# AzureLeon1/DiffSpectra

Measured on AMD Instinct MI355X. Metric: molecules/sec, 1000-step QM9S all-spectra sampling (partial run), higher is better.
Workload: dtype f32 (GEMMs as split-fp16 x3 MFMA with fp32 accumulate; fp32-level accuracy, parity gates unchanged)

## Files before the change

diffspectra_amd/csrc/ds_device.h:

```cpp
#pragma once
#include <hip/hip_runtime.h>
#include <stdint.h>

typedef float f32x16 __attribute__((ext_vector_type(16)));
typedef float f32x2 __attribute__((ext_vector_type(2)));
typedef _Float16 h4 __attribute__((ext_vector_type(4)));
typedef _Float16 h8 __attribute__((ext_vector_type(8)));
typedef float f32x4 __attribute__((ext_vector_type(4)));

#define DS_LDP 4

__device__ __forceinline__ float ds_silu(float x) { return __fdividef(x, 1.0f + __expf(-x)); }
__device__ __forceinline__ float ds_tanh(float x) {
  const float e = __builtin_amdgcn_exp2f(x * 2.8853900817779268f);
  return fmaf(-2.0f, __builtin_amdgcn_rcpf(e + 1.0f), 1.0f);
}
__device__ __forceinline__ f32x2 ds_tanh2_prescaled(f32x2 t) {
  f32x2 e;
  e.x = __builtin_amdgcn_exp2f(t.x); e.y = __builtin_amdgcn_exp2f(t.y);
  const f32x2 d = e + 1.0f;
  f32x2 r;
  r.x = __builtin_amdgcn_rcpf(d.x); r.y = __builtin_amdgcn_rcpf(d.y);
  return r * -2.0f + 1.0f;
}
// ... 191 lines not shown
  int voff;
  int kstride;
  int pstride;
};
__device__ __forceinline__ WStreamH wstream_h(const float* __restrict__ Wh, int N, int K, int col0) {
  const int lane = threadIdx.x & 63;
  WStreamH w;
  const unsigned long long pw = reinterpret_cast<unsigned long long>(Wh);
  const unsigned long long pu = (static_cast<unsigned long long>(__builtin_amdgcn_readfirstlane(static_cast<int>(pw >> 32))) << 32) |
                                static_cast<unsigned int>(__builtin_amdgcn_readfirstlane(static_cast<int>(pw)));
  w.rsrc = __builtin_amdgcn_make_buffer_rsrc(reinterpret_cast<float*>(pu), 0, 0x7fffffff, 0x00020000);
  w.voff = ((lane >> 5) * N + col0 + (lane & 31)) << 4;
  w.kstride = N << 5;
  w.pstride = (K >> 4) * w.kstride;
  return w;
}
__device__ __forceinline__ h8 wload_h(const WStreamH& w, int plane, int kb) {
  return __builtin_bit_cast(h8, __builtin_amdgcn_raw_buffer_load_b128(w.rsrc, w.voff, plane * w.pstride + kb * w.kstride, 0));
}

template <int MT, bool TRANS = false, int UNROLL = 4, bool XPF = true>
__device__ __forceinline__ void wave_mma_h(const _Float16* X, int K_tile, const float* __restrict__ Wh, int N, int K, int col0,
                                           int kb0, int kb1, f32x16 (&hi)[MT], f32x16 (&lo)[MT], int xkb0 = 0) {
  const int lane = threadIdx.x & 63, r = lane & 31, hh = lane >> 5;
  const int ldh = 2 * K_tile + 8;
  const WStreamH ws = wstream_h(Wh, N, K, col0);
  const _Float16* xr = X + r * ldh + 8 * hh - xkb0 * 16;
  h8 w1 = wload_h(ws, 0, kb0), w2 = wload_h(ws, 1, kb0);
  h8 xa[MT][2];
#pragma unroll
  for (int m = 0; m < MT; ++m) {
    xa[m][0] = *reinterpret_cast<const h8*>(xr + m * 32 * ldh + kb0 * 16);
    xa[m][1] = *reinterpret_cast<const h8*>(xr + m * 32 * ldh + K_tile + kb0 * 16);
  }
#pragma unroll UNROLL
  for (int kb = kb0; kb < kb1; ++kb) {
    const int kn = min(kb + 1, kb1 - 1);
    const h8 w1n = wload_h(ws, 0, kn), w2n = wload_h(ws, 1, kn);
    h8 xn[MT][2];
    if (XPF) {
#pragma unroll
      for (int m = 0; m < MT; ++m) {
        xn[m][0] = *reinterpret_cast<const h8*>(xr + m * 32 * ldh + kn * 16);
        xn[m][1] = *reinterpret_cast<const h8*>(xr + m * 32 * ldh + K_tile + kn * 16);
      }
    }
    __builtin_amdgcn_sched_barrier(0);
#pragma unroll
    for (int m = 0; m < MT; ++m) {
      if (TRANS) {
        hi[m] = __builtin_amdgcn_mfma_f32_32x32x16_f16(w1, xa[m][0], hi[m], 0, 0, 0);
        lo[m] = __builtin_amdgcn_mfma_f32_32x32x16_f16(w1, xa[m][1], lo[m], 0, 0, 0);
        lo[m] = __builtin_amdgcn_mfma_f32_32x32x16_f16(w2, xa[m][0], lo[m], 0, 0, 0);
      } else {
        hi[m] = __builtin_amdgcn_mfma_f32_32x32x16_f16(xa[m][0], w1, hi[m], 0, 0, 0);
        lo[m] = __builtin_amdgcn_mfma_f32_32x32x16_f16(xa[m][1], w1, lo[m], 0, 0, 0);
        lo[m] = __builtin_amdgcn_mfma_f32_32x32x16_f16(xa[m][0], w2, lo[m], 0, 0, 0);
      }
    }
    w1 = w1n; w2 = w2n;
#pragma unroll
    for (int m = 0; m < MT; ++m) {
      if (XPF) { xa[m][0] = xn[m][0]; xa[m][1] = xn[m][1]; }
      else {
        xa[m][0] = *reinterpret_cast<const h8*>(xr + m * 32 * ldh + kn * 16);
        xa[m][1] = *reinterpret_cast<const h8*>(xr + m * 32 * ldh + K_tile + kn * 16);
      }
    }
  }
}
constexpr int DS_MMA_XD = 1;
template <int PF>
struct WRingH {
  h8 w1[PF], w2[PF];
};
template <int PF>
__device__ __forceinline__ void wring_h(WRingH<PF>& ring, const WStreamH& ws, int kb0) {
#pragma unroll
  for (int i = 0; i < PF; ++i) {
    ring.w1[i] = wload_h(ws, 0, kb0 + i); ring.w2[i] = wload_h(ws, 1, kb0 + i);
    __builtin_amdgcn_sched_barrier(0);
  }
}
template <int MT, bool TRANS, int NKB, int PF, int XD = DS_MMA_XD>
__device__ __forceinline__ void wave_mma_h_deep(const _Float16* X, int K_tile, const WStreamH& ws, WRingH<PF>& ring, int kb0,
                                                f32x16 (&hi)[MT], f32x16 (&lo)[MT], int xkb0 = 0) {
  static_assert(PF <= NKB && XD <= NKB, "ring deeper than the product");
  const int lane = threadIdx.x & 63, r = lane & 31, hh = lane >> 5;
  const int ldh = 2 * K_tile + 8;
  const _Float16* xr = X + r * ldh + 8 * hh + (kb0 - xkb0) * 16;
  h8 xq[XD][MT][2];
#pragma unroll
  for (int d = 0; d < XD; ++d)
#pragma unroll
    for (int m = 0; m < MT; ++m) {
      xq[d][m][0] = *reinterpret_cast<const h8*>(xr + m * 32 * ldh + d * 16);
      xq[d][m][1] = *reinterpret_cast<const h8*>(xr + m * 32 * ldh + K_tile + d * 16);
    }
#pragma unroll
  for (int i = 0; i < NKB; ++i) {
    __builtin_amdgcn_sched_barrier(0);
    const h8 w1 = ring.w1[i % PF], w2 = ring.w2[i % PF];
    h8 xa[MT][2];
#pragma unroll
    for (int m = 0; m < MT; ++m) { xa[m][0] = xq[i % XD][m][0]; xa[m][1] = xq[i % XD][m][1]; }
#define DS_MMA_(ACC, WV, XV) ACC = TRANS ? __builtin_amdgcn_mfma_f32_32x32x16_f16(WV, XV, ACC, 0, 0, 0) : __builtin_amdgcn_mfma_f32_32x32x16_f16(XV, WV, ACC, 0, 0, 0)
#pragma unroll
    for (int m = 0; m < MT; ++m) DS_MMA_(lo[m], w1, xa[m][1]);
#pragma unroll
    for (int m = 0; m < MT; ++m) DS_MMA_(hi[m], w1, xa[m][0]);
#pragma unroll
    for (int m = 0; m < MT; ++m) DS_MMA_(lo[m], w2, xa[m][0]);
#undef DS_MMA_
    if (i + PF < NKB) {
      ring.w1[i % PF] = wload_h(ws, 0, kb0 + i + PF);
      ring.w2[i % PF] = wload_h(ws, 1, kb0 + i + PF);
    }
    if (i + XD < NKB) {
#pragma unroll
      for (int m = 0; m < MT; ++m) {
        xq[i % XD][m][0] = *reinterpret_cast<const h8*>(xr + m * 32 * ldh + (i + XD) * 16);
        xq[i % XD][m][1] = *reinterpret_cast<const h8*>(xr + m * 32 * ldh + K_tile + (i + XD) * 16);
      }
    }
    __builtin_amdgcn_sched_barrier(0);
  }
}
template <int MT, bool TRANS, int NKB, int PF>
__device__ __forceinline__ void wave_mma_h_deep_t2(const _Float16* X, int K_tile, const WStreamH& wsA, const WStreamH& wsB,
                                                   WRingH<PF>& ringA, WRingH<PF>& ringB, int kb0, f32x16 (&hiA)[MT], f32x16 (&loA)[MT],
                                                   f32x16 (&hiB)[MT], f32x16 (&loB)[MT], int xkb0 = 0) {
  static_assert(PF <= NKB, "ring deeper than the product");
  const int lane = threadIdx.x & 63, r = lane & 31, hh = lane >> 5;
  const int ldh = 2 * K_tile + 8;
  const _Float16* xr = X + r * ldh + 8 * hh + (kb0 - xkb0) * 16;
  h8 xa[MT][2];
#pragma unroll
  for (int m = 0; m < MT; ++m) {
    xa[m][0] = *reinterpret_cast<const h8*>(xr + m * 32 * ldh);
    xa[m][1] = *reinterpret_cast<const h8*>(xr + m * 32 * ldh + K_tile);
  }
#define DS_MMA_(ACC, WV, XV) ACC = TRANS ? __builtin_amdgcn_mfma_f32_32x32x16_f16(WV, XV, ACC, 0, 0, 0) : __builtin_amdgcn_mfma_f32_32x32x16_f16(XV, WV, ACC, 0, 0, 0)
#pragma unroll
  for (int i = 0; i < NKB; ++i) {
    const int in = i + 1 < NKB ? i + 1 : i;
    h8 xn[MT][2];
#pragma unroll
    for (int m = 0; m < MT; ++m) {
      xn[m][0] = *reinterpret_cast<const h8*>(xr + m * 32 * ldh + in * 16);
      xn[m][1] = *reinterpret_cast<const h8*>(xr + m * 32 * ldh + K_tile + in * 16);
    }
    __builtin_amdgcn_sched_barrier(0);
    const h8 a1 = ringA.w1[i % PF], a2 = ringA.w2[i % PF], b1 = ringB.w1[i % PF], b2 = ringB.w2[i % PF];
#pragma unroll
    for (int m = 0; m < MT; ++m) { DS_MMA_(loA[m], a1, xa[m][1]); DS_MMA_(loB[m], b1, xa[m][1]); }
#pragma unroll
    for (int m = 0; m < MT; ++m) { DS_MMA_(hiA[m], a1, xa[m][0]); DS_MMA_(hiB[m], b1, xa[m][0]); }
#pragma unroll
    for (int m = 0; m < MT; ++m) { DS_MMA_(loA[m], a2, xa[m][0]); DS_MMA_(loB[m], b2, xa[m][0]); }
    if (i + PF < NKB) {
      ringA.w1[i % PF] = wload_h(wsA, 0, kb0 + i + PF); ringA.w2[i % PF] = wload_h(wsA, 1, kb0 + i + PF);
      ringB.w1[i % PF] = wload_h(wsB, 0, kb0 + i + PF); ringB.w2[i % PF] = wload_h(wsB, 1, kb0 + i + PF);
    }
    __builtin_amdgcn_sched_barrier(0);
#pragma unroll
    for (int m = 0; m < MT; ++m) { xa[m][0] = xn[m][0]; xa[m][1] = xn[m][1]; }
  }
#undef DS_MMA_
}
template <int MT, bool TRANS, int NKB, int PF>
__device__ __forceinline__ void wave_mma_h_ring_t2(const _Float16* X, int K_tile, const WStreamH& wsA, const WStreamH& wsB, int kb0,
                                                   f32x16 (&hiA)[MT], f32x16 (&loA)[MT], f32x16 (&hiB)[MT], f32x16 (&loB)[MT], int xkb0 = 0) {
  WRingH<PF> ringA, ringB;
#pragma unroll
  for (int i = 0; i < PF; ++i) {
    ringA.w1[i] = wload_h(wsA, 0, kb0 + i); ringA.w2[i] = wload_h(wsA, 1, kb0 + i);
    ringB.w1[i] = wload_h(wsB, 0, kb0 + i); ringB.w2[i] = wload_h(wsB, 1, kb0 + i);
    __builtin_amdgcn_sched_barrier(0);
  }
  wave_mma_h_deep_t2<MT, TRANS, NKB, PF>(X, K_tile, wsA, wsB, ringA, ringB, kb0, hiA, loA, hiB, loB, xkb0);
}

template <int MT, bool TRANS, int NKB, int PF>
__device__ __forceinline__ void wave_mma_h_ring(const _Float16* X, int K_tile, const float* __restrict__ Wh, int N, int K, int col0,
                                                int kb0, f32x16 (&hi)[MT], f32x16 (&lo)[MT], int xkb0 = 0) {
  const WStreamH ws = wstream_h(Wh, N, K, col0);
  WRingH<PF> ring;
  wring_h<PF>(ring, ws, kb0);
  wave_mma_h_deep<MT, TRANS, NKB, PF>(X, K_tile, ws, ring, kb0, hi, lo, xkb0);
}
template <int MT>
__device__ __forceinline__ void split_finish(f32x16 (&hi)[MT], const f32x16 (&lo)[MT]) {
#pragma unroll
  for (int m = 0; m < MT; ++m)
#pragma unroll
    for (int i = 0; i < 16; ++i) hi[m][i] = fmaf(lo[m][i], 1.0f / 2048.0f, hi[m][i]);
}

template <int MT>
__device__ __forceinline__ void acc_zero(f32x16 (&acc)[MT]) {
#pragma unroll
  for (int m = 0; m < MT; ++m)
#pragma unroll
    for (int i = 0; i < 16; ++i) acc[m][i] = 0.0f;
}

// ... 89 lines not shown
```

diffspectra_amd/csrc/ds_kernels.hip:

```cpp
#include <hip/hip_runtime.h>
#include <math.h>
#include <stdint.h>
#include <stdio.h>
#include <stdlib.h>

#include <atomic>
#include <mutex>
#include <utility>
#include <vector>

#include "../../include/diffspectra_hip.h"
#include "ds_device.h"
#include "ds_train_common.h"

#define ADAC DS_ADA_COLS
constexpr int DS_NODE_PF = 8;
constexpr int DS_NODE_PF2 = 4;
constexpr int DS_QKV_PF = 4;
constexpr int DS_TWO_STREAM_MAX_PAIRS = 400000;

#ifdef DS_STAMPS
#define DS_STAMP_INIT()                                                                                 \
  unsigned long long _sa[16] = {0, 0, 0, 0, 0, 0, 0, 0, 0, 0, 0, 0, 0, 0, 0, 0};                        \
  unsigned long long _t0 = __builtin_amdgcn_s_memtime()
// ... 96 lines not shown
      const int d = c.L.node_dense[row];
      if (k < 6) v = xh[(size_t)d * 9 + 3 + k];
      else if (k < 12) v = cond_x ? cond_x[(size_t)d * 9 + 3 + (k - 6)] : 0.0f;
      else if (k < 15) v = xh[(size_t)d * 9 + (k - 12)];
    }
    in[rr][k] = v;
  }
  __syncthreads();
  const float* W = GW(c, DS_GW_NODE_EMB_W);
  float w[12];
#pragma unroll
  for (int k = 0; k < 12; ++k) w[k] = wp_at(W, 256, k, col);
  const float bias = GW(c, DS_GW_NODE_EMB_B)[col];
#pragma unroll
  for (int rr = 0; rr < R; ++rr) {
    const int row = row0 + rr;
    if (row >= c.L.Nn) break;
    float acc = 0.0f;
#pragma unroll
    for (int k = 0; k < 12; ++k) acc += in[rr][k] * w[k];
    acc += bias;
    c.ws.h[(size_t)row * 256 + col] = acc;
    c.ws.atom_hids[(size_t)row * 768 + col] = acc;
    if (col < 4) c.ws.pos[(size_t)row * 4 + col] = col < 3 ? in[rr][12 + col] : 0.0f;
  }
}

__global__ __launch_bounds__(256) void k_pair_init(Ctx c, const float* __restrict__ edge_x, const float* __restrict__ cond_x,
                                                   const float* __restrict__ cond_edge_x) {
  ds_fp16_saturate();
  constexpr int T = 64;
  __shared__ __attribute__((aligned(16))) float X[T][72 + DS_LDP];
  __shared__ __attribute__((aligned(16))) float xs[T];
  const int tid = threadIdx.x, row0 = blockIdx.x * T;
  const bool use_rbf = (cond_x != nullptr) && (c.ws.flags[0] != 0);
  if (tid < T) {
    const int p = row0 + tid;
    float x = 0.0f;
    float e0 = 0, e1 = 0, c0 = 0, c1 = 0;
    if (p < c.L.Pp) {
      const int da = c.L.node_dense[c.L.pair_a[p]], db = c.L.node_dense[c.L.pair_b[p]];
      const int m = c.L.pair_mol[p];
      const size_t eidx = ((size_t)da * c.L.N + (db - m * c.L.N)) * 2;
      e0 = edge_x[eidx]; e1 = edge_x[eidx + 1];
      if (cond_x != nullptr) {
        c0 = cond_edge_x[eidx]; c1 = cond_edge_x[eidx + 1];
        const float* pa = cond_x + (size_t)da * 9;
        const float* pb = cond_x + (size_t)db * 9;
        const float dx = pa[0] - pb[0], dy = pa[1] - pb[1], dz = pa[2] - pb[2];
        const float d2 = dx * dx + dy * dy + dz * dz;
        const float* ad = c.ws.ada + (size_t)m * ADAC + DS_ADA_TOP;
        x = use_rbf ? d2 * (ad[0] + 1.0f) + ad[1] : d2;
      }
    }
    X[tid][0] = e0; X[tid][1] = e1; X[tid][2] = c0; X[tid][3] = c1;
    X[tid][68] = 0.0f; X[tid][69] = 0.0f; X[tid][70] = 0.0f; X[tid][71] = 0.0f;
    xs[tid] = x;
  }
  __syncthreads();
  const float* mean = GW(c, DS_GW_RBF_MEAN);
  const float* stdv = GW(c, DS_GW_RBF_STD);
  const float* astd = GW(c, DS_GW_RBF_ASTD);
  for (int idx = tid; idx < T * 64; idx += 256) {
    const int row = idx >> 6, k = idx & 63;
    float v = 0.0f;
    if (row0 + row < c.L.Pp) v = use_rbf ? rbf_feature(xs[row], k, mean, stdv, astd) : xs[row];
    X[row][4 + k] = v;
  }
  __syncthreads();
  const float* bias = GW(c, DS_GW_EDGE_EMB_B);
  const int Pp = c.L.Pp;
  float* e = c.ws.e;
  float* hid = c.ws.edge_hids;
  tile_gemm<2, 1>(&X[0][0], 72 + DS_LDP, 72, GW(c, DS_GW_EDGE_EMB_W), 64, 2, [&](int row, int col, float v) {
    const int p = row0 + row;
    if (p < Pp) {
      const float y = v + bias[col];
      e[(size_t)p * 64 + col] = y;
      hid[(size_t)p * 192 + col] = y;
    }
  });
}

__global__ __launch_bounds__(256) void k_edge_geom(Ctx c, int blk) {
  ds_fp16_saturate();
  constexpr int T = 64, LDH = 2 * 128 + 8;
  __shared__ __attribute__((aligned(16))) _Float16 Xh[T][LDH];
  __shared__ __attribute__((aligned(16))) float Y[T][64 + DS_LDP];
  __shared__ __attribute__((aligned(16))) float xs[T];
  __shared__ int rmol[T];
  const int tid = threadIdx.x, row0 = blockIdx.x * T;
  const int kf = tid & 63, rbp = tid >> 6;
  const float mk = kf ? BW(c, blk, DS_BW_RBF_MEAN)[kf - 1] : 0.0f;
  const float sk = kf ? BW(c, blk, DS_BW_RBF_STD)[kf - 1] : 1.0f;
  const float ak = kf ? BW(c, blk, DS_BW_RBF_ASTD)[kf - 1] : 1.0f;
  float ev[16];
#pragma unroll
  for (int j = 0; j < 16; ++j) ev[j] = c.ws.e[(size_t)min(row0 + rbp + 4 * j, c.L.Pp - 1) * 64 + kf];
  if (tid < T) {
    const int p = row0 + tid;
    float x = 0.0f;
    int m = 0;
    if (p < c.L.Pp) {
      m = c.L.pair_mol[p];
      const float* pa = c.ws.pos + (size_t)c.L.pair_a[p] * 4;
      const float* pb = c.ws.pos + (size_t)c.L.pair_b[p] * 4;
      const float dx = pa[0] - pb[0], dy = pa[1] - pb[1], dz = pa[2] - pb[2];
      const float d2 = dx * dx + dy * dy + dz * dz;
      const float* ad = c.ws.ada + (size_t)m * ADAC + blk * DS_ADA_BLOCK_STRIDE + DS_ADA_DIST;
      x = d2 * (ad[0] + 1.0f) + ad[1];
    }
    xs[tid] = x;
    rmol[tid] = m;
    if (p < c.L.Pp) c.ws.dist[p] = x;
  }
  __syncthreads();
  float4 lsh[4], lsc[4];
  {
    const float* ade = c.ws.ada + blk * DS_ADA_BLOCK_STRIDE + DS_ADA_EDGE;
    const int lane = tid & 63, wv = tid >> 6;
#pragma unroll
    for (int j = 0; j < 4; ++j) {
      const float* am = ade + (size_t)rmol[16 * wv + 4 * j + (lane >> 4)] * ADAC;
      lsh[j] = reinterpret_cast<const float4*>(am)[lane & 15];
      lsc[j] = reinterpret_cast<const float4*>(am + 64)[lane & 15];
    }
  }
  {
    const int k = kf, rb = rbp;
    const float rsk = __builtin_amdgcn_rcpf(sk), rak = __builtin_amdgcn_rcpf(ak);
    const int Pp = c.L.Pp;
#pragma unroll
    for (int j = 0; j < 16; ++j) {
      const int row = rb + 4 * j, p = row0 + row;
      const float x = xs[row];
      const float z = (x - mk) * rsk;
      float v = k ? __expf(-0.5f * (z * z)) * rak : x;
      if (p >= Pp) { v = 0.0f; ev[j] = 0.0f; }
      split_store1(&Xh[row][0], 128, k, v);
      split_store1(&Xh[row][0], 128, 64 + k, ev[j]);
    }
  }
  {
    const int wv = tid >> 6, mt = wv >> 1, cc = wv & 1, lane = tid & 63;
    const WStreamH wse = wstream_h(BW(c, blk, DS_BW_EDGE_EMB_H), 64, 128, cc * 32);
    WRingH<8> ring;
    wring_h<8>(ring, wse, 0);
    const float bcol = BW(c, blk, DS_BW_EDGE_EMB_B)[cc * 32 + (lane & 31)];
    __syncthreads();
    f32x16 acc[1], lo[1];
#pragma unroll
    for (int i = 0; i < 16; ++i) acc[0][i] = bcol;
    acc_zero<1>(lo);
    wave_mma_h_deep<1, false, 8, 8>(&Xh[mt * 32][0], 128, wse, ring, 0, acc, lo);
    split_finish<1>(acc, lo);
#pragma unroll
    for (int i = 0; i < 16; ++i) Y[mt * 32 + acc_row(i, lane >> 5)][cc * 32 + (lane & 31)] = acc[0][i];
  }
  __syncthreads();
  {
    const int lane = tid & 63, wv = tid >> 6;
    _Float16* ye = reinterpret_cast<_Float16*>(c.ws.ye);
#pragma unroll
    for (int j = 0; j < 4; ++j) {
      const int row = 16 * wv + 4 * j + (lane >> 4);
      const float4 v = ln_mod_reg64(reinterpret_cast<const float4*>(&Y[row][0])[lane & 15], lsh[j], lsc[j]);
      if (row0 + row < c.L.Pp) split_store4(ye + (size_t)(row0 + row) * 128, 64, 4 * (lane & 15), v);
    }
  }
}

template <int NW>
__global__ __launch_bounds__(NW * 64) void k_node_qkv(Ctx c, int blk) {
  ds_fp16_saturate();
  constexpr int NT = NW * 64;
  constexpr int T = 64;
  constexpr int LDH = 2 * 256 + 8;
  __shared__ __attribute__((aligned(16))) _Float16 Xh[T][LDH];
  __shared__ int rmol[T];
  const int tid = threadIdx.x, row0 = blockIdx.x * T, col0 = blockIdx.y * 384;
  if (tid < T) rmol[tid] = (row0 + tid < c.L.Nn) ? c.L.node_mol[row0 + tid] : 0;
  __syncthreads();
  {
    const float* adn = c.ws.ada + blk * DS_ADA_BLOCK_STRIDE + DS_ADA_NODE;
    const int lane = tid & 63, wv = tid >> 6, g = lane >> 4, j = lane & 15;
    static_assert(NT == 256, "four waves x 16 rows");
#pragma unroll
    for (int half = 0; half < 2; ++half) {
      float4 v[2][4], sh[2][4], sc[2][4];
#pragma unroll
      for (int ps = 0; ps < 2; ++ps) {
        const int row = 16 * wv + 8 * half + 4 * ps + g;
        const float4* hp = reinterpret_cast<const float4*>(c.ws.h + (size_t)min(row0 + row, c.L.Nn - 1) * 256) + j;
        const float4* ap = reinterpret_cast<const float4*>(adn + (size_t)rmol[row] * ADAC) + j;
#pragma unroll
        for (int u = 0; u < 4; ++u) {
          v[ps][u] = hp[16 * u];
          sh[ps][u] = ap[16 * u];
          sc[ps][u] = ap[64 + 16 * u];
        }
      }
#pragma unroll
      for (int ps = 0; ps < 2; ++ps) {
        const int row = 16 * wv + 8 * half + 4 * ps + g;
        ln_mod_quad256(v[ps], sh[ps], sc[ps]);
#pragma unroll
        for (int u = 0; u < 4; ++u)
          split_store4(&Xh[row][0], 256, 64 * u + 4 * j, row0 + row < c.L.Nn ? v[ps][u] : make_float4(0, 0, 0, 0));
      }
    }
  }
  __syncthreads();
  const float* bias = BW(c, blk, DS_BW_QKV_B) + col0;
  float* qkv = c.ws.qkv + (size_t)row0 * 768 + col0;
  const int valid = c.L.Nn - row0, wave = tid >> 6;
  for (int ch = wave; ch < 12; ch += NW) {
    asm volatile("" ::: "memory");
    const float b = bias[ch * 32 + (tid & 31)];
    f32x16 acc[2], lo[2];
#pragma unroll
    for (int m = 0; m < 2; ++m)
#pragma unroll
      for (int i = 0; i < 16; ++i) acc[m][i] = b;
    acc_zero<2>(lo);
    wave_mma_h_ring<2, false, 16, DS_QKV_PF>(&Xh[0][0], 256, BW(c, blk, DS_BW_QKV_H), 768, 256, col0 + ch * 32, 0, acc, lo);
    split_finish<2>(acc, lo);
    acc_store<2, 768>(acc, qkv + ch * 32, valid, [](int, float v) { return v; });
  }
}

__global__ __launch_bounds__(1024) void k_attn_fused(Ctx c, int blk) {
  ds_fp16_saturate();
  DS_STAMP_INIT();
  constexpr int NT = 1024, QS = 512 + 32, LDT = 256 + 4, LDY = 2 * 64 + 8, CR = 32, MAXP = DS_MAX_ATOMS * (DS_MAX_ATOMS - 1) / 2;
  __shared__ __attribute__((aligned(16))) float QK[DS_MAX_ATOMS * QS];
  __shared__ __attribute__((aligned(16))) float Tt[2][CR][LDT];
  __shared__ __attribute__((aligned(16))) _Float16 Yc[2][CR][LDY];
  __shared__ __attribute__((aligned(16))) float AL[2][CR][32];
  __shared__ int PT[(MAXP + 15) & ~15];
  __shared__ int VT[32][32];
  static_assert(DS_MAX_ATOMS <= 32 && MAXP <= 511 - CR, "visit table packing");
  static_assert(DS_MAX_ATOMS * 128 <= 4 * NT && DS_MAX_ATOMS * 64 <= 2 * NT && MAXP <= NT, "single-pass staging");
  const int tid = threadIdx.x, wave = tid >> 6, lane = tid & 63, hh = lane >> 5;
  int n0, n, p0, P;
  if (c.L.mol_by_size) {
    const int4 r = reinterpret_cast<const int4*>(c.L.mol_by_size)[blockIdx.x];
    n0 = r.x; n = r.y; p0 = r.z; P = r.w;
  } else {
    const int m = blockIdx.x;
    n0 = c.L.node_off[m]; n = c.L.node_off[m + 1] - n0;
    p0 = c.L.pair_off[m]; P = c.L.pair_off[m + 1] - p0;
// ... 1033 lines not shown
    for (int u = 0; u < 8; ++u) {
      const int idx = i0 + u * 256, row = idx / 192, k4 = idx - row * 192;
      v[u] = reinterpret_cast<const float4*>(c.ws.atom_hids + (size_t)min(row0 + row, Nn - 1) * 768)[k4];
    }
#pragma unroll
    for (int u = 0; u < 8; ++u) {
      const int idx = i0 + u * 256, row = idx / 192, k4 = idx - row * 192;
      split_store4(&X[row][0], 768, 4 * k4, row0 + row < Nn ? v[u] : make_float4(0, 0, 0, 0));
    }
  }
  __syncthreads();
  {
    const float* b = GW(c, DS_GW_NP0_B);
    for (int ch = wave; ch < 8; ch += 4) {
      asm volatile("" ::: "memory");
      const int col = ch * 32 + (tid & 31), hhf = (tid & 63) >> 5;
      const float bc = b[col];
      f32x16 acc[1], lo[1];
#pragma unroll
      for (int i = 0; i < 16; ++i) acc[0][i] = bc;
      acc_zero<1>(lo);
      wave_mma_h_ring<1, false, 48, 8>(&X[0][0], 768, GW(c, DS_GW_NP0_H), 256, 768, ch * 32, 0, acc, lo);
      split_finish<1>(acc, lo);
#pragma unroll
      for (int i = 0; i < 16; ++i) split_store1(&Y1[acc_row(i, hhf)][0], 256, col, ds_silu(acc[0][i]));
    }
  }
  __syncthreads();
  {
    const float* b = GW(c, DS_GW_NP2_B);
    const int col = wave * 32 + (tid & 31), hhf = (tid & 63) >> 5;
    const float bc = b[col];
    f32x16 acc[1], lo[1];
#pragma unroll
    for (int i = 0; i < 16; ++i) acc[0][i] = bc;
    acc_zero<1>(lo);
    wave_mma_h_ring<1, false, 16, 8>(&Y1[0][0], 256, GW(c, DS_GW_NP2_H), 128, 256, wave * 32, 0, acc, lo);
    split_finish<1>(acc, lo);
#pragma unroll
    for (int i = 0; i < 16; ++i) Y2[acc_row(i, hhf)][col] = ds_silu(acc[0][i]);
  }
  __syncthreads();
  {
    const float* b = GW(c, DS_GW_NP4_B);
    const float bc = b[min((int)(threadIdx.x & 31), 5)];
    tile_gemm<1, 1>(&Y2[0][0], 128 + DS_LDP, 128, GW(c, DS_GW_NP4_W), 32, 1, [&](int row, int col, float v) {
      if (col < 6 && dn[row] >= 0) out_xh[(size_t)dn[row] * 9 + 3 + col] = v + bc;
    });
  }
}

__global__ __launch_bounds__(256) void k_edge_readout(Ctx c, float* __restrict__ out_edge) {
  ds_fp16_saturate();
  const int tid = threadIdx.x, wave = tid >> 6, lane = tid & 63, r = lane & 31, hh = lane >> 5;
  const int Pp = c.L.Pp;
  const int row0 = (blockIdx.x * 4 + wave) * 32;
  if (row0 >= Pp) return;
  const int p = min(row0 + r, Pp - 1);
  const bool valid = row0 + r < Pp;
  const int pa = c.L.pair_a[p], pb = c.L.pair_b[p], pm = c.L.pair_mol[p];
  h8 x1[12], x2[12];
  {
    const float4* src = reinterpret_cast<const float4*>(c.ws.edge_hids + (size_t)p * 192 + 8 * hh);
#pragma unroll
    for (int g4 = 0; g4 < 3; ++g4) {
      float4 v[4][2];
#pragma unroll
      for (int u = 0; u < 4; ++u) { v[u][0] = src[(g4 * 4 + u) * 4]; v[u][1] = src[(g4 * 4 + u) * 4 + 1]; }
#pragma unroll
      for (int u = 0; u < 4; ++u) {
        const float xs[8] = {v[u][0].x, v[u][0].y, v[u][0].z, v[u][0].w, v[u][1].x, v[u][1].y, v[u][1].z, v[u][1].w};
#pragma unroll
        for (int t = 0; t < 8; ++t) {
          const _Float16 a1 = (_Float16)xs[t];
          x1[g4 * 4 + u][t] = a1;
          x2[g4 * 4 + u][t] = (_Float16)((xs[t] - (float)a1) * 2048.0f);
        }
      }
    }
  }
  const int da = c.L.node_dense[pa], db = c.L.node_dense[pb];
  const int mN = pm * c.L.N;
  const size_t oab = ((size_t)da * c.L.N + (db - mN)) * 2, oba = ((size_t)db * c.L.N + (da - mN)) * 2;
  for (int ch = 0; ch < 2; ++ch) {
    const int g0 = ch == 0 ? DS_GW_EX0_W : DS_GW_ET0_W;
    const float* b0 = GW(c, g0 + 1);
    const float* b2 = GW(c, g0 + 3);
    const uint4* W2 = reinterpret_cast<const uint4*>(GW(c, ch == 0 ? DS_GW_EX2_C : DS_GW_ET2_C)) + lane;
    f32x16 a2, a2lo;
#pragma unroll
    for (int q = 0; q < 4; ++q) {
      const float4 bb = *reinterpret_cast<const float4*>(b2 + 8 * q + 4 * hh);
      a2[4 * q] = bb.x; a2[4 * q + 1] = bb.y; a2[4 * q + 2] = bb.z; a2[4 * q + 3] = bb.w;
    }
#pragma unroll
    for (int i = 0; i < 16; ++i) a2lo[i] = 0.0f;
#pragma unroll
    for (int hc = 0; hc < 2; ++hc) {
      asm volatile("" ::: "memory");
      const WStreamH ws0 = wstream_h(GW(c, ch == 0 ? DS_GW_EX0_H : DS_GW_ET0_H), 64, 192, hc * 32);
      WRingH<6> ring;
      wring_h<6>(ring, ws0, 0);
      f32x16 a1, a1lo;
#pragma unroll
      for (int q = 0; q < 4; ++q) {
        const float4 bb = *reinterpret_cast<const float4*>(b0 + hc * 32 + 8 * q + 4 * hh);
        a1[4 * q] = bb.x; a1[4 * q + 1] = bb.y; a1[4 * q + 2] = bb.z; a1[4 * q + 3] = bb.w;
      }
#pragma unroll
      for (int i = 0; i < 16; ++i) a1lo[i] = 0.0f;
#pragma unroll
      for (int kb = 0; kb < 12; ++kb) {
        const h8 w1 = ring.w1[kb % 6], w2 = ring.w2[kb % 6];
        a1lo = __builtin_amdgcn_mfma_f32_32x32x16_f16(w1, x2[kb], a1lo, 0, 0, 0);
        a1 = __builtin_amdgcn_mfma_f32_32x32x16_f16(w1, x1[kb], a1, 0, 0, 0);
        a1lo = __builtin_amdgcn_mfma_f32_32x32x16_f16(w2, x1[kb], a1lo, 0, 0, 0);
        if (kb + 6 < 12) { ring.w1[kb % 6] = wload_h(ws0, 0, kb + 6); ring.w2[kb % 6] = wload_h(ws0, 1, kb + 6); }
        __builtin_amdgcn_sched_barrier(0);
      }
#pragma unroll
      for (int i = 0; i < 16; ++i) a1[i] = fmaf(a1lo[i], 1.0f / 2048.0f, a1[i]);
#pragma unroll
      for (int s_ = 0; s_ < 2; ++s_) {
        h8 y1, y2;
#pragma unroll
        for (int j = 0; j < 8; j += 2) {
          f32x2 v;
          v.x = a1[8 * s_ + j]; v.y = a1[8 * s_ + j + 1];
          v = ds_silu2(v);
          y1[j] = (_Float16)v.x; y1[j + 1] = (_Float16)v.y;
          y2[j] = (_Float16)((v.x - (float)y1[j]) * 2048.0f); y2[j + 1] = (_Float16)((v.y - (float)y1[j + 1]) * 2048.0f);
        }
        const h8 w1 = __builtin_bit_cast(h8, W2[((0 * 2 + hc) * 2 + s_) * 64]);
        const h8 w2 = __builtin_bit_cast(h8, W2[((1 * 2 + hc) * 2 + s_) * 64]);
        a2 = __builtin_amdgcn_mfma_f32_32x32x16_f16(w1, y1, a2, 0, 0, 0);
        a2lo = __builtin_amdgcn_mfma_f32_32x32x16_f16(w1, y2, a2lo, 0, 0, 0);
        a2lo = __builtin_amdgcn_mfma_f32_32x32x16_f16(w2, y1, a2lo, 0, 0, 0);
      }
    }
    const float* W4 = GW(c, g0 + 4);
    f32x2 s2 = {0.0f, 0.0f};
#pragma unroll
    for (int i = 0; i < 16; i += 2) {
      f32x2 v;
      v.x = fmaf(a2lo[i], 1.0f / 2048.0f, a2[i]); v.y = fmaf(a2lo[i + 1], 1.0f / 2048.0f, a2[i + 1]);
      v = ds_silu2(v);
      const f32x2 w = {wp_at(W4, 32, acc_row(i, hh), 0), wp_at(W4, 32, acc_row(i + 1, hh), 0)};
      s2 = __builtin_elementwise_fma(w, v, s2);
    }
    const float part = s2.x + s2.y;
    const auto sw = __builtin_amdgcn_permlane32_swap(__float_as_uint(part), __float_as_uint(part), false, false);
    const float val = (__uint_as_float(sw[0]) + __uint_as_float(sw[1])) + GW(c, g0 + 5)[0];
    if (valid && hh == 0) {
      out_edge[oab + ch] = val;
      out_edge[oba + ch] = val;
    }
  }
}

__global__ void k_final_pos(Ctx c, float* __restrict__ out_xh) {
  const int m = blockIdx.x * blockDim.x + threadIdx.x;
  if (m >= c.L.B) return;
  const int n0 = c.L.node_off[m], n = c.L.node_off[m + 1] - n0;
  const bool nan = c.ws.flags[1] != 0;
  float sx = 0.0f, sy = 0.0f, sz = 0.0f;
  for (int a = 0; a < n; ++a) {
    const float* pp = c.ws.pos + (size_t)(n0 + a) * 4;
    if (!nan) { sx += pp[0]; sy += pp[1]; sz += pp[2]; }
  }
  const float fn = (float)n;
  for (int a = 0; a < n; ++a) {
    const float* pp = c.ws.pos + (size_t)(n0 + a) * 4;
    float* o = out_xh + (size_t)c.L.node_dense[n0 + a] * 9;
    const float px = nan ? 0.0f : pp[0], py = nan ? 0.0f : pp[1], pz = nan ? 0.0f : pp[2];
    o[0] = px - sx / fn; o[1] = py - sy / fn; o[2] = pz - sz / fn;
  }
}

__global__ void k_temb_finish(Ctx c, const float* __restrict__ tm3, int tm3_rows, const float* __restrict__ ctx) {
  ds_fp16_saturate();
  const size_t i = (size_t)blockIdx.x * blockDim.x + threadIdx.x;
  if (i >= (size_t)c.L.B * 1024) return;
  const size_t b = i >> 10, col = i & 1023;
  float v = tm3[(tm3_rows == 1 ? 0 : b) * 1024 + col];
  if (ctx) v += ctx[i];
  split_store1(reinterpret_cast<_Float16*>(c.ws.temb_silu) + b * 2048, 1024, (int)col, ds_silu(v));
}

__global__ __launch_bounds__(256) void k_gemm_ada(const _Float16* __restrict__ A, const float* __restrict__ Wh, const float* __restrict__ bias,
                                                  float* __restrict__ C, int ldc, int M, int K, int N) {
  ds_fp16_saturate();
  constexpr int T = 64, KC = 64, LDH = 2 * KC + 8, MT = T / 32;
  __shared__ __attribute__((aligned(16))) _Float16 X[2][T][LDH];
  const int tid = threadIdx.x, wave = tid >> 6;
  const int row0 = blockIdx.x * T;
  const int col0 = (blockIdx.y * 4 + wave) * 32;
  const bool active = col0 < N;
  const int nchunks = K / KC;
  float4 st0, st1, st2, st3;
  const int srow = tid >> 4, spiece = tid & 15;
  const size_t scol = (size_t)(spiece >> 3) * K + (spiece & 7) * 8;
  auto fetch = [&](int kc) {
    const _Float16* base = A + scol + kc * KC;
    st0 = *reinterpret_cast<const float4*>(base + (size_t)min(row0 + srow, M - 1) * 2 * K);
    st1 = *reinterpret_cast<const float4*>(base + (size_t)min(row0 + srow + 16, M - 1) * 2 * K);
    st2 = *reinterpret_cast<const float4*>(base + (size_t)min(row0 + srow + 32, M - 1) * 2 * K);
    st3 = *reinterpret_cast<const float4*>(base + (size_t)min(row0 + srow + 48, M - 1) * 2 * K);
  };
  auto stash = [&](int buf) {
    *reinterpret_cast<float4*>(&X[buf][srow][spiece * 8]) = st0;
    *reinterpret_cast<float4*>(&X[buf][srow + 16][spiece * 8]) = st1;
    *reinterpret_cast<float4*>(&X[buf][srow + 32][spiece * 8]) = st2;
    *reinterpret_cast<float4*>(&X[buf][srow + 48][spiece * 8]) = st3;
  };
  f32x16 acc[MT], lo[MT];
  acc_zero<MT>(acc);
  acc_zero<MT>(lo);
  const WStreamH wsw = wstream_h(Wh, N, K, active ? col0 : 0);
  WRingH<4> ring;
  wring_h<4>(ring, wsw, 0);
  fetch(0);
  stash(0);
  __syncthreads();
  for (int kc = 0; kc < nchunks; ++kc) {
    const int cur = kc & 1;
    if (kc + 1 < nchunks) fetch(kc + 1);
    if (active) wave_mma_h_deep<MT, false, 4, 4>(&X[cur][0][0], KC, wsw, ring, kc * 4, acc, lo, kc * 4);
    if (kc + 1 < nchunks) { wring_h<4>(ring, wsw, kc * 4 + 4); stash(cur ^ 1); }
    __syncthreads();
  }
  if (!active) return;
  split_finish<MT>(acc, lo);
  const int lane = tid & 63, r = lane & 31, hh = lane >> 5, col = col0 + r;
  const float bcol = bias ? bias[col] : 0.0f;
  const unsigned long long pw = reinterpret_cast<unsigned long long>(C + (size_t)row0 * ldc + col0);
  const unsigned long long pu = (static_cast<unsigned long long>(__builtin_amdgcn_readfirstlane(static_cast<int>(pw >> 32))) << 32) |
                                static_cast<unsigned int>(__builtin_amdgcn_readfirstlane(static_cast<int>(pw)));
  const __amdgpu_buffer_rsrc_t rc = __builtin_amdgcn_make_buffer_rsrc(reinterpret_cast<float*>(pu), 0, 0x7fffffff, 0x00020000);
// ... 428 lines not shown
    if (kc + 1 < nchunks) fetch(kc + 1);
    const float* wp = g.Wp + (size_t)(kc * (KC / 8)) * 2 * g.Npad * 4;
    if (active) wave_mma<4>(&X[cur][0][0], LD, wp, g.Npad, col0, 0, KC / 8, acc, 0, &bf);
    if (kc + 1 < nchunks) {
      stash(cur ^ 1);
      bf = bfrag_load(wp + (size_t)(KC / 8) * 2 * g.Npad * 4, g.Npad, active ? col0 : 0, 0, 8);
    }
    __syncthreads();
  }
  if (!active) return;
  {
    const int lane = tid & 63, r = lane & 31, hh = lane >> 5, col = col0 + r;
    const bool colok = col < g.N;
    const float bcol = (g.bias && colok) ? g.bias[col] : 0.0f;
    const float csc = (g.cs && colok) ? g.cs[col] : 1.0f, csh = (g.cs && colok) ? g.csh[col] : 0.0f;
    const unsigned long long pw = reinterpret_cast<unsigned long long>(g.C + (size_t)row0 * g.ldc + col0);
    const unsigned long long pu = (static_cast<unsigned long long>(__builtin_amdgcn_readfirstlane(static_cast<int>(pw >> 32))) << 32) |
                                  static_cast<unsigned int>(__builtin_amdgcn_readfirstlane(static_cast<int>(pw)));
    const __amdgpu_buffer_rsrc_t rc = __builtin_amdgcn_make_buffer_rsrc(reinterpret_cast<float*>(pu), 0, 0x7fffffff, 0x00020000);
    const int voff = (4 * hh * g.ldc + r) * 4, rowb = g.ldc * 4;
#pragma unroll
    for (int m = 0; m < 4; ++m)
#pragma unroll
      for (int i = 0; i < 16; ++i) {
        const int row = m * 32 + (i & 3) + 8 * (i >> 2), gr = row0 + row + 4 * hh;
        if (gr < g.M && colok) {
          float v = ds_act<ACT>(acc[m][i] + bcol);
          if (g.R) v += g.R[(size_t)(g.r_grp_rows > 0 ? gr % g.r_grp_rows : gr) * g.ldr + col];
          if (g.cs) v = v * csc + csh;
          __builtin_amdgcn_raw_buffer_store_b32(__float_as_uint(v), rc, voff, row * rowb, 0);
        }
      }
  }
}

int gemm_dispatch(const GemmArgs& g, int act, hipStream_t s) {
  if (!g.A || !g.Wp || !g.C || g.M <= 0 || g.K <= 0 || g.N <= 0 || (g.cs && !g.csh)) return DS_ERR_ARG;
  const bool big = g.M >= 512 && g.a_grp_rows <= 0 && g.c_grp_rows <= 0 && g.K % 64 == 0 && g.lda % 4 == 0 &&
                   (reinterpret_cast<uintptr_t>(g.A) & 15) == 0;
  using Kernel = void (*)(GemmArgs);
  static constexpr Kernel tile128[4] = {k_gemm_big<0>, k_gemm_big<1>, k_gemm_big<2>, k_gemm_big<3>};
  static constexpr Kernel tile64[4] = {k_gemm<0>, k_gemm<1>, k_gemm<2>, k_gemm<3>};
  if (act < 0 || act > 3) return DS_ERR_ARG;
  const int rows = big ? 128 : 64;
  hipLaunchKernelGGL(big ? tile128[act] : tile64[act], dim3((g.M + rows - 1) / rows, (g.Npad + 127) / 128), dim3(256), 0, s, g);
  return DST_CHECK_LAUNCH();
}

int gemm_simple(const float* A, int64_t lda, const float* Wp, const float* bias, float* C, int64_t ldc, int M, int K, int N,
                int act, int a_silu, hipStream_t s) {
  GemmArgs g{};
  g.A = A; g.lda = lda; g.Wp = Wp; g.bias = bias; g.C = C; g.ldc = ldc; g.M = M; g.K = K; g.N = N;
  g.Npad = (N + 31) & ~31; g.a_silu = a_silu;
  return gemm_dispatch(g, act, s);
}

enum ProfSlot { PROF_EDGE_GEOM = 0, PROF_NODE_QKV = 1, PROF_ATTN = 2, PROF_NODE_UPDATE = 3, PROF_EDGE_UPDATE = 4, PROF_EQUI_PAIRS = 5 };
struct ProfState {
  int kernel = -1;
  int every = 1;
  long long seen = 0;
  std::vector<std::pair<hipEvent_t, hipEvent_t>> pool;
  size_t used = 0;
};
ProfState g_prof;

struct ProfScope {
  hipStream_t s;
  bool on = false;
  ProfScope(int kernel, hipStream_t st) : s(st) {
    if (g_prof.kernel != kernel) return;
    if ((g_prof.seen++ % g_prof.every) != 0 || g_prof.used >= g_prof.pool.size()) return;
    on = true;
    (void)hipEventRecord(g_prof.pool[g_prof.used].first, s);
  }
  ~ProfScope() {
    if (on) (void)hipEventRecord(g_prof.pool[g_prof.used++].second, s);
  }
};

void launch_edge_geom(const Ctx& c, int blk, hipStream_t s) {
  if (c.L.Pp <= 0) return;
  ProfScope ps(PROF_EDGE_GEOM, s);
  hipLaunchKernelGGL(k_edge_geom, dim3((c.L.Pp + 63) / 64), dim3(256), 0, s, c, blk);
}
void launch_node_qkv(const Ctx& c, int blk, hipStream_t s) {
  ProfScope ps(PROF_NODE_QKV, s);
  hipLaunchKernelGGL(k_node_qkv<4>, dim3((c.L.Nn + 63) / 64, 2), dim3(256), 0, s, c, blk);
}
void launch_attn(const Ctx& c, int blk, hipStream_t s) {
  ProfScope ps(PROF_ATTN, s);
  hipLaunchKernelGGL(k_attn_fused, dim3(c.L.B), dim3(1024), 0, s, c, blk);
}
void launch_node_n2e(const Ctx& c, int blk, hipStream_t s) { hipLaunchKernelGGL(k_node_n2e, dim3((c.L.Nn + 63) / 64), dim3(256), 0, s, c, blk); }
template <bool N2E>
void launch_node_update(const Ctx& c, int blk, hipStream_t s) {
  ProfScope ps(PROF_NODE_UPDATE, s);
  hipLaunchKernelGGL(k_node_update<N2E>, dim3((c.L.Nn + 31) / 32), dim3(256), 0, s, c, blk);
}
void launch_edge_update(const Ctx& c, int blk, hipStream_t s) {
  if (c.L.Pp <= 0) return;
  ProfScope ps(PROF_EDGE_UPDATE, s);
  hipLaunchKernelGGL(k_edge_update, dim3((c.L.Pp + 127) / 128), dim3(256), 0, s, c, blk);
}
void launch_equi_pairs(const Ctx& c, int blk, hipStream_t s) {
  if (c.L.Pp <= 0) return;
  ProfScope ps(PROF_EQUI_PAIRS, s);
  hipLaunchKernelGGL(k_equi_pairs, dim3(min((c.L.Pp + 31) / 32, device_cus())), dim3((EQUI_NCW + EQUI_NLW) * 64), 0, s, c, blk);
}
void launch_pos_update(const Ctx& c, int last, hipStream_t s) { hipLaunchKernelGGL(k_pos_update, dim3(c.L.B), dim3(64), 0, s, c, last); }

}

extern "C" {

void ds_struct_sizes(int64_t* out) {
  out[0] = sizeof(ds_weights);
  out[1] = sizeof(ds_layout);
  out[2] = sizeof(ds_workspace);
  out[3] = sizeof(ds_gemm_args);
}

int ds_gemm(const ds_gemm_args* a, void* stream) {
  if (!a) return DS_ERR_ARG;
  GemmArgs g{};
  g.A = a->A; g.lda = a->lda; g.a_grp_rows = a->a_grp_rows; g.a_grp_stride = a->a_grp_stride;
  g.Wp = a->Wp; g.bias = a->bias;
  g.C = a->C; g.ldc = a->ldc; g.c_grp_rows = a->c_grp_rows; g.c_grp_stride = a->c_grp_stride;
  g.M = a->M; g.K = a->K; g.N = a->N; g.Npad = (a->N + 31) & ~31;
  g.R = a->R; g.ldr = a->ldr; g.r_grp_rows = a->r_grp_rows;
  g.cs = a->col_scale; g.csh = a->col_shift; g.a_silu = a->a_silu;
  return gemm_dispatch(g, a->act, (hipStream_t)stream);
}

int ds_gemm_split(const void* A_split, const float* W_split, const float* bias, float* C, int64_t ldc, int32_t M, int32_t K,
                  int32_t N, void* stream) {
  if (!A_split || !W_split || !C || M <= 0 || K <= 0 || N <= 0 || K % 64 != 0 || N % 32 != 0 || ldc < N) return DS_ERR_ARG;
  hipLaunchKernelGGL(k_gemm_ada, dim3((M + 63) / 64, (N + 127) / 128), dim3(256), 0, (hipStream_t)stream,
                     reinterpret_cast<const _Float16*>(A_split), W_split, bias, C, (int)ldc, M, K, N);
  return DST_CHECK_LAUNCH();
}

int ds_stage_time(const ds_weights* w, const ds_layout* L, ds_workspace* ws, const float* noise_level, const float* ctx_emb,
                  void* stream) {
  hipStream_t s = (hipStream_t)stream;
  Ctx c;
  if (!make_ctx(c, w, L, ws) || !noise_level) return DS_ERR_ARG;
  const int B = L->B;
  const int64_t* off = w->off + DS_NBLOCKS * DS_W_BLOCK_SLOTS;
  hipLaunchKernelGGL(k_time_feat, dim3((B + 63) / 64), dim3(64), 0, s, c, noise_level);
  int st = gemm_simple(ws->tfeat, 24, w->base + off[DS_GW_TM1_W], w->base + off[DS_GW_TM1_B], ws->tmid, 1024, B, 24, 1024, 2, 0, s);
  if (st) return st;
  float* tm3 = ws->ada;
  st = gemm_simple(ws->tmid, 1024, w->base + off[DS_GW_TM3_W], w->base + off[DS_GW_TM3_B], tm3, 1024, B, 1024, 1024, 0, 0, s);
  if (st) return st;
  const size_t tot = (size_t)B * 1024;
  hipLaunchKernelGGL(k_temb_finish, dim3((unsigned)((tot + 255) / 256)), dim3(256), 0, s, c, (const float*)tm3, B, ctx_emb);
  static_assert(ADAC % 32 == 0, "adaLN table width");
  return ds_gemm_split(ws->temb_silu, w->base + off[DS_GW_ADA_W], w->base + off[DS_GW_ADA_B], ws->ada, ADAC, B, 1024, ADAC, stream);
}

int ds_stage_init(const ds_weights* w, const ds_layout* L, ds_workspace* ws, const float* xh, const float* edge_x,
                  const float* cond_x, const float* cond_edge_x, void* stream) {
  hipStream_t s = (hipStream_t)stream;
  Ctx c;
  if (!make_ctx(c, w, L, ws) || !xh || !edge_x || ((cond_x == nullptr) != (cond_edge_x == nullptr))) return DS_ERR_ARG;
  if (!clear(ws->flags, 8 * sizeof(int32_t), s)) return DS_ERR_LAUNCH;
// ... 221 lines not shown
```

Measured before the change: 233.6.

## Make edge_geom kernel persistent with software-pipelined prefetch of next tile

Turns k_edge_geom into a persistent kernel: the grid is capped at 3 workgroups per CU, and each block walks a contiguous range of 64-row tiles. While the current tile is being processed, the block prefetches the next tile's edge features, positions and ada coefficients, plus the pair indices two tiles ahead. The per-thread work layout changes to vectorized float4 RBF/split stores, and the adaLN loads are issued during the MFMA loop, whose accumulators are pinned to keep them in registers. The edge-output kernel also merges its two scalar channel stores into one float2 store, at the cost of more register pressure and a longer per-block loop.

```diff
diff --git a/diffspectra_amd/csrc/ds_device.h b/diffspectra_amd/csrc/ds_device.h
--- a/diffspectra_amd/csrc/ds_device.h
+++ b/diffspectra_amd/csrc/ds_device.h
@@ -297,7 +297,7 @@
     __builtin_amdgcn_sched_barrier(0);
   }
 }
-template <int MT, bool TRANS, int NKB, int PF, int XD = DS_MMA_XD>
+template <int MT, bool TRANS, int NKB, int PF, int XD = DS_MMA_XD, bool PIN = false>
 __device__ __forceinline__ void wave_mma_h_deep(const _Float16* X, int K_tile, const WStreamH& ws, WRingH<PF>& ring, int kb0,
                                                 f32x16 (&hi)[MT], f32x16 (&lo)[MT], int xkb0 = 0) {
   static_assert(PF <= NKB && XD <= NKB, "ring deeper than the product");
@@ -337,6 +337,10 @@
         xq[i % XD][m][0] = *reinterpret_cast<const h8*>(xr + m * 32 * ldh + (i + XD) * 16);
         xq[i % XD][m][1] = *reinterpret_cast<const h8*>(xr + m * 32 * ldh + K_tile + (i + XD) * 16);
       }
+    }
+    if (PIN) {
+#pragma unroll
+      for (int m = 0; m < MT; ++m) asm volatile("" : "+v"(hi[m]), "+v"(lo[m]));
     }
     __builtin_amdgcn_sched_barrier(0);
   }
diff --git a/diffspectra_amd/csrc/ds_kernels.hip b/diffspectra_amd/csrc/ds_kernels.hip
--- a/diffspectra_amd/csrc/ds_kernels.hip
+++ b/diffspectra_amd/csrc/ds_kernels.hip
@@ -202,91 +202,127 @@
   });
 }
 
-__global__ __launch_bounds__(256) void k_edge_geom(Ctx c, int blk) {
+constexpr int EG_WGS_PER_CU = 3;
+constexpr int EG_PF = 4;
+struct EdgeGeomIdx {
+  int a, b, m;
+};
+struct EdgeGeomRows {
+  float4 e[4];
+  float4 pa, pb;
+  float ad0, ad1;
+  int m;
+};
+__device__ __forceinline__ void edge_geom_idx(EdgeGeomIdx& ix, const Ctx& c, int row0) {
+  const int p = min(row0 + 16 * (int)(threadIdx.x >> 6) + (int)(threadIdx.x & 15), c.L.Pp - 1);
+  ix.a = c.L.pair_a[p]; ix.b = c.L.pair_b[p]; ix.m = c.L.pair_mol[p];
+}
+__device__ __forceinline__ void edge_geom_request(EdgeGeomRows& r, const Ctx& c, int blk, int row0, const EdgeGeomIdx& ix) {
+  const int lane = threadIdx.x & 63, wv = threadIdx.x >> 6;
+#pragma unroll
+  for (int i = 0; i < 4; ++i)
+    r.e[i] = reinterpret_cast<const float4*>(c.ws.e + (size_t)min(row0 + 16 * wv + (lane >> 4) + 4 * i, c.L.Pp - 1) * 64)[lane & 15];
+  r.pa = *reinterpret_cast<const float4*>(c.ws.pos + (size_t)ix.a * 4);
+  r.pb = *reinterpret_cast<const float4*>(c.ws.pos + (size_t)ix.b * 4);
+  const float* ad = c.ws.ada + (size_t)ix.m * ADAC + blk * DS_ADA_BLOCK_STRIDE + DS_ADA_DIST;
+  r.ad0 = ad[0]; r.ad1 = ad[1];
+  r.m = ix.m;
+}
+__global__ __launch_bounds__(256, EG_WGS_PER_CU) void k_edge_geom(Ctx c, int blk) {
   ds_fp16_saturate();
   constexpr int T = 64, LDH = 2 * 128 + 8;
   __shared__ __attribute__((aligned(16))) _Float16 Xh[T][LDH];
   __shared__ __attribute__((aligned(16))) float Y[T][64 + DS_LDP];
-  __shared__ __attribute__((aligned(16))) float xs[T];
-  __shared__ int rmol[T];
-  const int tid = threadIdx.x, row0 = blockIdx.x * T;
-  const int kf = tid & 63, rbp = tid >> 6;
-  const float mk = kf ? BW(c, blk, DS_BW_RBF_MEAN)[kf - 1] : 0.0f;
-  const float sk = kf ? BW(c, blk, DS_BW_RBF_STD)[kf - 1] : 1.0f;
-  const float ak = kf ? BW(c, blk, DS_BW_RBF_ASTD)[kf - 1] : 1.0f;
-  float ev[16];
-#pragma unroll
-  for (int j = 0; j < 16; ++j) ev[j] = c.ws.e[(size_t)min(row0 + rbp + 4 * j, c.L.Pp - 1) * 64 + kf];
-  if (tid < T) {
-    const int p = row0 + tid;
-    float x = 0.0f;
-    int m = 0;
-    if (p < c.L.Pp) {
-      m = c.L.pair_mol[p];
-      const float* pa = c.ws.pos + (size_t)c.L.pair_a[p] * 4;
-      const float* pb = c.ws.pos + (size_t)c.L.pair_b[p] * 4;
-      const float dx = pa[0] - pb[0], dy = pa[1] - pb[1], dz = pa[2] - pb[2];
+  const int tid = threadIdx.x, lane = tid & 63, wv = tid >> 6;
+  const int Pp = c.L.Pp;
+  const int nt = (Pp + T - 1) / T;
+  const int t0 = (int)((long long)blockIdx.x * nt / gridDim.x), t1 = (int)((long long)(blockIdx.x + 1) * nt / gridDim.x);
+  if (t0 >= t1) return;
+  const int jq = lane & 15, rq = lane >> 4;
+  float mk[4], rsk[4], rak[4];
+#pragma unroll
+  for (int u = 0; u < 4; ++u) {
+    const int kf = 4 * jq + u;
+    mk[u] = kf ? BW(c, blk, DS_BW_RBF_MEAN)[kf - 1] : 0.0f;
+    rsk[u] = __builtin_amdgcn_rcpf(kf ? BW(c, blk, DS_BW_RBF_STD)[kf - 1] : 1.0f);
+    rak[u] = __builtin_amdgcn_rcpf(kf ? BW(c, blk, DS_BW_RBF_ASTD)[kf - 1] : 1.0f);
+  }
+  const int mt = wv >> 1, cc = wv & 1;
+  const WStreamH wse = wstream_h(BW(c, blk, DS_BW_EDGE_EMB_H), 64, 128, cc * 32);
+  const float bcol = BW(c, blk, DS_BW_EDGE_EMB_B)[cc * 32 + (lane & 31)];
+  const float* ade = c.ws.ada + blk * DS_ADA_BLOCK_STRIDE + DS_ADA_EDGE;
+  _Float16* ye = reinterpret_cast<_Float16*>(c.ws.ye);
+  EdgeGeomIdx ix;
+  EdgeGeomRows r;
+  edge_geom_idx(ix, c, t0 * T);
+  edge_geom_request(r, c, blk, t0 * T, ix);
+  edge_geom_idx(ix, c, min(t0 + 1, t1 - 1) * T);
+  for (int t = t0; t < t1; ++t) {
+    const int row0 = t * T;
+    float xr[4];
+    int mr[4];
+    {
+      const float dx = r.pa.x - r.pb.x, dy = r.pa.y - r.pb.y, dz = r.pa.z - r.pb.z;
       const float d2 = dx * dx + dy * dy + dz * dz;
-      const float* ad = c.ws.ada + (size_t)m * ADAC + blk * DS_ADA_BLOCK_STRIDE + DS_ADA_DIST;
-      x = d2 * (ad[0] + 1.0f) + ad[1];
-    }
-    xs[tid] = x;
-    rmol[tid] = m;
-    if (p < c.L.Pp) c.ws.dist[p] = x;
-  }
-  __syncthreads();
-  float4 lsh[4], lsc[4];
-  {
-    const float* ade = c.ws.ada + blk * DS_ADA_BLOCK_STRIDE + DS_ADA_EDGE;
-    const int lane = tid & 63, wv = tid >> 6;
-#pragma unroll
-    for (int j = 0; j < 4; ++j) {
-      const float* am = ade + (size_t)rmol[16 * wv + 4 * j + (lane >> 4)] * ADAC;
-      lsh[j] = reinterpret_cast<const float4*>(am)[lane & 15];
-      lsc[j] = reinterpret_cast<const float4*>(am + 64)[lane & 15];
-    }
-  }
-  {
-    const int k = kf, rb = rbp;
-    const float rsk = __builtin_amdgcn_rcpf(sk), rak = __builtin_amdgcn_rcpf(ak);
-    const int Pp = c.L.Pp;
-#pragma unroll
-    for (int j = 0; j < 16; ++j) {
-      const int row = rb + 4 * j, p = row0 + row;
-      const float x = xs[row];
-      const float z = (x - mk) * rsk;
-      float v = k ? __expf(-0.5f * (z * z)) * rak : x;
-      if (p >= Pp) { v = 0.0f; ev[j] = 0.0f; }
-      split_store1(&Xh[row][0], 128, k, v);
-      split_store1(&Xh[row][0], 128, 64 + k, ev[j]);
-    }
-  }
-  {
-    const int wv = tid >> 6, mt = wv >> 1, cc = wv & 1, lane = tid & 63;
-    const WStreamH wse = wstream_h(BW(c, blk, DS_BW_EDGE_EMB_H), 64, 128, cc * 32);
-    WRingH<8> ring;
-    wring_h<8>(ring, wse, 0);
-    const float bcol = BW(c, blk, DS_BW_EDGE_EMB_B)[cc * 32 + (lane & 31)];
+      const float x = d2 * (r.ad0 + 1.0f) + r.ad1;
+      const int p = row0 + 16 * wv + jq;
+      if (rq == 0 && p < Pp) c.ws.dist[p] = x;
+#pragma unroll
+      for (int i = 0; i < 4; ++i) {
+        xr[i] = __shfl(x, rq + 4 * i);
+        mr[i] = __shfl(r.m, rq + 4 * i);
+      }
+    }
+#pragma unroll
+    for (int i = 0; i < 4; ++i) {
+      const int row = 16 * wv + rq + 4 * i;
+      const bool in = row0 + row < Pp;
+      const float x = xr[i];
+      float v[4];
+#pragma unroll
+      for (int u = 0; u < 4; ++u) {
+        const float z = (x - mk[u]) * rsk[u];
+        const float gk = __expf(-0.5f * (z * z)) * rak[u];
+        v[u] = (u == 0 && jq == 0) ? x : gk;
+      }
+      split_store4(&Xh[row][0], 128, 4 * jq, in ? make_float4(v[0], v[1], v[2], v[3]) : make_float4(0, 0, 0, 0));
+      split_store4(&Xh[row][0], 128, 64 + 4 * jq, in ? r.e[i] : make_float4(0, 0, 0, 0));
+    }
+    __builtin_amdgcn_sched_barrier(0);
+    WRingH<EG_PF> ring;
+    wring_h<EG_PF>(ring, wse, 0);
+    edge_geom_request(r, c, blk, min(t + 1, t1 - 1) * T, ix);
+    edge_geom_idx(ix, c, min(t + 2, t1 - 1) * T);
+    __builtin_amdgcn_sched_barrier(0);
     __syncthreads();
-    f32x16 acc[1], lo[1];
-#pragma unroll
-    for (int i = 0; i < 16; ++i) acc[0][i] = bcol;
-    acc_zero<1>(lo);
-    wave_mma_h_deep<1, false, 8, 8>(&Xh[mt * 32][0], 128, wse, ring, 0, acc, lo);
-    split_finish<1>(acc, lo);
-#pragma unroll
-    for (int i = 0; i < 16; ++i) Y[mt * 32 + acc_row(i, lane >> 5)][cc * 32 + (lane & 31)] = acc[0][i];
-  }
-  __syncthreads();
-  {
-    const int lane = tid & 63, wv = tid >> 6;
-    _Float16* ye = reinterpret_cast<_Float16*>(c.ws.ye);
-#pragma unroll
-    for (int j = 0; j < 4; ++j) {
-      const int row = 16 * wv + 4 * j + (lane >> 4);
-      const float4 v = ln_mod_reg64(reinterpret_cast<const float4*>(&Y[row][0])[lane & 15], lsh[j], lsc[j]);
-      if (row0 + row < c.L.Pp) split_store4(ye + (size_t)(row0 + row) * 128, 64, 4 * (lane & 15), v);
-    }
+    float4 lsh[4], lsc[4];
+    {
+      f32x16 acc[1], lo[1];
+      float bc = bcol;
+      asm volatile("" : "+v"(bc));
+#pragma unroll
+      for (int i = 0; i < 16; ++i) acc[0][i] = bc;
+      acc_zero<1>(lo);
+      wave_mma_h_deep<1, false, 8, EG_PF, DS_MMA_XD, true>(&Xh[mt * 32][0], 128, wse, ring, 0, acc, lo);
+#pragma unroll
+      for (int i = 0; i < 4; ++i) {
+        const float* am = ade + (size_t)mr[i] * ADAC;
+        lsh[i] = reinterpret_cast<const float4*>(am)[jq];
+        lsc[i] = reinterpret_cast<const float4*>(am + 64)[jq];
+      }
+      split_finish<1>(acc, lo);
+#pragma unroll
+      for (int i = 0; i < 16; ++i) Y[mt * 32 + acc_row(i, lane >> 5)][cc * 32 + (lane & 31)] = acc[0][i];
+    }
+    __syncthreads();
+    __builtin_amdgcn_sched_barrier(0);
+#pragma unroll
+    for (int i = 0; i < 4; ++i) {
+      const int row = 16 * wv + 4 * i + rq;
+      const float4 v = ln_mod_reg64(reinterpret_cast<const float4*>(&Y[row][0])[jq], lsh[i], lsc[i]);
+      if (row0 + row < Pp) split_store4(ye + (size_t)(row0 + row) * 128, 64, 4 * jq, v);
+    }
+    __builtin_amdgcn_sched_barrier(0);
   }
 }
 
@@ -1486,6 +1522,7 @@
   const int da = c.L.node_dense[pa], db = c.L.node_dense[pb];
   const int mN = pm * c.L.N;
   const size_t oab = ((size_t)da * c.L.N + (db - mN)) * 2, oba = ((size_t)db * c.L.N + (da - mN)) * 2;
+  float val0 = 0.0f;
   for (int ch = 0; ch < 2; ++ch) {
     const int g0 = ch == 0 ? DS_GW_EX0_W : DS_GW_ET0_W;
     const float* b0 = GW(c, g0 + 1);
@@ -1555,9 +1592,10 @@
     const float part = s2.x + s2.y;
     const auto sw = __builtin_amdgcn_permlane32_swap(__float_as_uint(part), __float_as_uint(part), false, false);
     const float val = (__uint_as_float(sw[0]) + __uint_as_float(sw[1])) + GW(c, g0 + 5)[0];
-    if (valid && hh == 0) {
-      out_edge[oab + ch] = val;
-      out_edge[oba + ch] = val;
+    if (ch == 0) val0 = val;
+    else if (valid && hh == 0) {
+      *reinterpret_cast<float2*>(out_edge + oab) = make_float2(val0, val);
+      *reinterpret_cast<float2*>(out_edge + oba) = make_float2(val0, val);
     }
   }
 }
@@ -2152,7 +2190,7 @@
 void launch_edge_geom(const Ctx& c, int blk, hipStream_t s) {
   if (c.L.Pp <= 0) return;
   ProfScope ps(PROF_EDGE_GEOM, s);
-  hipLaunchKernelGGL(k_edge_geom, dim3((c.L.Pp + 63) / 64), dim3(256), 0, s, c, blk);
+  hipLaunchKernelGGL(k_edge_geom, dim3(min((c.L.Pp + 63) / 64, EG_WGS_PER_CU * device_cus())), dim3(256), 0, s, c, blk);
 }
 void launch_node_qkv(const Ctx& c, int blk, hipStream_t s) {
   ProfScope ps(PROF_NODE_QKV, s);
```

Measured after the change: 234.5 (median of 6 runs). Within noise of the previous version (+0.4%).
